# rbrito/deprecated-lame-mirror

Hardware: AMD Instinct MI355X
Metric: encoded audio seconds/sec (x real-time) at 44.1kHz stereo CBR128 (higher is better)
Workload: dtype f32

## Files before the change

### deprecated-lame-mirror_amd/csrc/lh_analysis.hip

```cpp
#include <stdint.h>
#include <math.h>

#ifdef LH_EMU
#include "hipemu.h"
#define LH_CONST static const
#else
#include <hip/hip_runtime.h>
#define LH_CONST __device__ static const
#endif

#if defined(LH_APROF) && !defined(LH_EMU)
__shared__ unsigned long long *lh_ap_base;
#define LH_PT(var) unsigned long long var = clock64()
#define LH_PA(idx, var) do { if (c.lane == 0) atomicAdd(&lh_ap_base[LH_NPROF * c.wave + 20 + (idx)], clock64() - var); } while (0)
#define LH_PC(idx) do { } while (0)
#endif
#define LH_CUSTOM_LDS "lh_lds_analysis.h"
#define LH_CUSTOM_SMP
#define LH_FZ_X(i) ((((i) >> 4) & 2) | (((i) >> 3) & 24) | (((i) >> 5) & 4))
#define LH_FZ(i) ((i) ^ LH_FZ_X(i))
#define LH_STAGE_IDX(i) LH_FZ(i)
#include "lh_static_tables.h"
#include "lh_dev_common.h"
#if !defined(LH_EMU)
#define LH_KRESTRICT __restrict__
#else
#define LH_KRESTRICT
#endif

#define LH_SPAN (lh_lds.work)
LH_DEVFN float
lh_smp(const LhCtx & c, int ch, int i)
{
    return LH_SPAN[ch * LH_BLKSIZE + LH_FZ(i)];
}

#include "lh_dev_psy_core.h"

struct LhGranuleAt {
    int     live;
    int     gr;
    long long at;
    long long frame_base;
};

LH_DEVFN LhGranuleAt
lh_granule_at(const LhStreamDesc & d, int g)
{
    LhGranuleAt o;
    int const nf = d.frame_end - d.frame_begin;
    int const fr = g / LH_NGR;
    o.live = g < LH_NGR * nf;
    o.gr = g - fr * LH_NGR;
    o.at = d.out_index + d.mid_rel + fr;
    o.frame_base = (long long) (576 * LH_NGR) * (d.frame_begin + fr) - LH_MF_START;
    return o;
}

LH_DEVFN LhStreamDesc
lh_desc_uniform(const LhStreamDesc * descs, int sidx)
{
    LhStreamDesc d = descs[sidx];
    d.pcm_l = lh_uni_ll(d.pcm_l);
    d.pcm_r = lh_uni_ll(d.pcm_r);
    d.pcm_base = lh_uni_ll(d.pcm_base);
    d.nsamples = lh_uni_ll(d.nsamples);
    d.out_index = lh_uni_ll(d.out_index);
    d.mid_rel = lh_uni_i(d.mid_rel);
    d.frame_begin = lh_uni_i(d.frame_begin);
    d.frame_end = lh_uni_i(d.frame_end);
    return d;
}

#ifdef LH_LSF
#define lh_attack_kernel lh_attack_kernel_lsf
#define lh_attack_scan_kernel lh_attack_scan_kernel_lsf
#define lh_analysis_kernel lh_analysis_kernel_lsf
#define lh_launch_analysis lh_launch_analysis_lsf
#define lh_emu_analysis lh_emu_analysis_lsf
#endif

#if defined(LH_APROF) && !defined(LH_EMU)
#define LH_AP_T0() unsigned long long ap_t = clock64()
#define LH_AP(k) do { unsigned long long const n_ = clock64(); if (c.lane == 0) atomicAdd(&aprof[64 * 0 + LH_NPROF * c.wave + (k)], n_ - ap_t); ap_t = n_; } while (0)
#else
#define LH_AP_T0() do { } while (0)
#define LH_AP(k) do { } while (0)
#endif
#define LH_FIR_SPAN 640

#ifndef LH_EMU
extern "C" __global__ void __launch_bounds__(64)
#else
void
#endif
lh_attack_kernel(const LhConfig * LH_KRESTRICT cfg, const int16_t * LH_KRESTRICT pcm, const float *pcmf, const LhStreamDesc * descs, LhMidFrame * frames,
                 int nstreams)
{
    __shared__ float span[2 * LH_FIR_SPAN];
    int const sidx = (int) blockIdx.y;
    LhCtx   c;
    c.cfg = cfg;
    c.T = nullptr;
    c.st = nullptr;
    c.pcm = pcm;
    c.pcmf = pcmf;
    c.d = lh_desc_uniform(descs, sidx);
    c.tid = (int) threadIdx.x;
    c.lane = c.tid;
    c.wave = 0;
    LhGranuleAt const ga = lh_granule_at(c.d, (int) blockIdx.x);
    if (!ga.live)
        return;
    int const lane = c.lane;
    int const n_chn_psy = (cfg->mode == LH_MODE_JOINT_STEREO) ? 4 : cfg->channels;
    int const bufbase = 576 + ga.gr * 576 - LH_FFTOFFSET;
    int const firbase = bufbase + 576 - 350 - LH_NSFIRLEN + 192;
    LhMidGr *mg = &frames[ga.at].small.gr[ga.gr];
    lh_stage_span < LH_FIR_SPAN, 64, 1 > (c, span, span + LH_FIR_SPAN, ga.frame_base + firbase);
    LH_WAVE_SYNC();
    {
        int const i0 = 9 * lane;
        float   x[2][30], y[2][9];
#pragma unroll
        for (int ch = 0; ch < 2; ch++)
#pragma unroll
            for (int t = 0; t < 30; t++)
                x[ch][t] = span[ch * LH_FIR_SPAN + i0 + t];
#pragma unroll
        for (int ch = 0; ch < 2; ch++)
#pragma unroll
            for (int m = 0; m < 9; m++) {
                float   sum1 = x[ch][m + 10], sum2 = 0.0;
#pragma unroll
                for (int j = 0; j < ((LH_NSFIRLEN - 1) / 2) - 1; j += 2) {
                    sum1 += lh_hp_fir[j] * (x[ch][m + j] + x[ch][m + LH_NSFIRLEN - j]);
                    sum2 += lh_hp_fir[j + 1] * (x[ch][m + j + 1] + x[ch][m + LH_NSFIRLEN - j - 1]);
                }
                y[ch][m] = sum1 + sum2;
            }
        LH_WAVE_SYNC();
#pragma unroll
        for (int ch = 0; ch < 2; ch++)
#pragma unroll
            for (int m = 0; m < 9; m++)
                span[ch * LH_FIR_SPAN + i0 + m] = y[ch][m];
    }
    LH_WAVE_SYNC();
    float   fl[9], fr[9];
#pragma unroll
    for (int k = 0; k < 9; k++) {
        fl[k] = span[lane + 64 * k];
        fr[k] = span[LH_FIR_SPAN + lane + 64 * k];
    }
    for (int chn = 0; chn < n_chn_psy; chn++) {
        uint32_t pk[8], pk8 = 0;
#pragma unroll
        for (int k = 0; k < 9; k++) {
            float const l = fl[k], r = fr[k];
            float const v = (chn == 0) ? l : (chn == 1) ? r : (chn == 2) ? l + r : l - r;
            if (k < 8)
                pk[k] = lh_f32_as_u32(lh_fabsf(v));
            else
                pk8 = lh_f32_as_u32(lh_fabsf(v));
        }
        {
            uint32_t const m8 = lh_wave_max8(pk);
            uint32_t const m9 = lh_wave_max_u32(pk8);
            if (lane < 9)
                mg->peak[chn][lane] = lh_u32_as_f32(lane == 8 ? m9 : m8);
        }
    }
}

#ifndef LH_SCAN_BLOCK
#define LH_SCAN_BLOCK 4
#endif
#ifndef LH_EMU
extern "C" __global__ void __launch_bounds__(64)
#else
void
#endif
lh_attack_scan_kernel(const LhConfig * LH_KRESTRICT cfg, const LhTables * LH_KRESTRICT T, const LhStreamDesc * descs, const LhStreamState * states,
                      LhMidFrame * frames, int nstreams)
{
    int const sidx = (int) blockIdx.x;
    int const lane = (int) threadIdx.x;
    LhStreamDesc const d = lh_desc_uniform(descs, sidx);
    int const nf = d.frame_end - d.frame_begin;
    if (nf <= 0)
        return;
    const LhStreamState *st = &states[sidx];
    int const n_chn_psy = lh_uni_i((cfg->mode == LH_MODE_JOINT_STEREO) ? 4 : cfg->channels);
    int const channels = lh_uni_i(cfg->channels), short_blocks = lh_uni_i(cfg->short_blocks);
    int const chn = lane >> 4, i = lane & 15, grp = lane & 48;
    int const mine = chn < n_chn_psy;
    float   le = st->last_en_subshort[chn][i < 9 ? i : 0];
    int     last_att = st->last_attacks[chn];
    float const thresh = T->attack_threshold[chn];
    int     bt_old0 = lh_uni_i(st->blocktype_old[0]), bt_old1 = lh_uni_i(st->blocktype_old[1]);
    int const ng = LH_NGR * nf;
    float   pk_blk[LH_SCAN_BLOCK];
#pragma unroll
    for (int j = 0; j < LH_SCAN_BLOCK; j++) {
        int const g = (j < ng) ? j : 0;
        pk_blk[j] = frames[d.out_index + d.mid_rel + g / LH_NGR].small.gr[g % LH_NGR].peak[chn][i < 9 ? i : 0];
    }
    for (int g0 = 0; g0 < ng; g0 += LH_SCAN_BLOCK) {
        float   pk_cur[LH_SCAN_BLOCK], ssf_blk[LH_SCAN_BLOCK];
        int     nsa_blk[LH_SCAN_BLOCK][4];
#pragma unroll
        for (int j = 0; j < LH_SCAN_BLOCK; j++) {
            int const gn = g0 + LH_SCAN_BLOCK + j, g = (gn < ng) ? gn : 0;
            pk_cur[j] = pk_blk[j];
            pk_blk[j] = frames[d.out_index + d.mid_rel + g / LH_NGR].small.gr[g % LH_NGR].peak[chn][i < 9 ? i : 0];
        }
#pragma unroll
        for (int j = 0; j < LH_SCAN_BLOCK; j++) {
            float const pk = pk_cur[j];
            float const fresh = pk < 1.0f ? 1.0f : pk;
            float const old = lh_shfl_f32(le, grp + ((i + 6) & 15)), older = lh_shfl_f32(le, grp + ((i + 4) & 15));
            float const got = lh_shfl_f32(fresh, grp + ((i - 3) & 15));
            float const e = (i < 3) ? old : got;
            float const e1 = lh_shfl_f32(e, grp + ((i - 1) & 15)), e0 = lh_shfl_f32(e, grp + ((i - 2) & 15));
            float const then = (i < 3) ? older : e0;
            float const ai = (i < 3) ? e / then : (e > then) ? e / then : (then > e * 10.0f) ? then / (e * 10.0f) : 0.0f;
            float const whole = e0 + e1 + e;
            int const tail_low = e * 6 < whole, mid_low = e1 * 6 < whole;
            uint64_t const over_all = lh_ballot(i < 12 && ai > thresh);
            unsigned const over = (unsigned) (over_all >> (16 * chn)) & 0xfffu;
            float   en_short[4];
            en_short[0] = lh_shfl_f32(whole, grp + 2);
            en_short[1] = lh_shfl_f32(whole, grp + 5);
            en_short[2] = lh_shfl_f32(whole, grp + 8);
            en_short[3] = lh_shfl_f32(whole, grp + 11);
            ssf_blk[j] = tail_low ? (mid_low ? 0.25f : 0.5f) : 1.0f;
            int    *nsa = nsa_blk[j];
            le = fresh;
            for (int gq = 0; gq < 4; gq++) {
                unsigned const bits = (over >> (3 * gq)) & 7u;
                nsa[gq] = bits ? ((bits & 1u) ? 1 : (bits & 2u) ? 2 : 3) : 0;
            }
            for (int q = 1; q < 4; q++) {
                float const u = en_short[q - 1];
                float const v = en_short[q];
                float const m = (u > v) ? u : v;
                if (m < 40000) {
                    if (u < 1.7f * v && v < 1.7f * u) {
                        if (q == 1 && nsa[0] <= nsa[q])
                            nsa[0] = 0;
                        nsa[q] = 0;
                    }
                }
            }
        }
#pragma unroll
        for (int j = 0; j < LH_SCAN_BLOCK; j++) {
            int const g = g0 + j;
            if (g >= ng)
                break;
            int const fr = g / LH_NGR, gr = g - fr * LH_NGR;
            LhMidGr *mg = &frames[d.out_index + d.mid_rel + fr].small.gr[gr];
            int    *nsa = nsa_blk[j];
            float const ssf = ssf_blk[j];
            int     uselong = 1;
            if (nsa[0] <= last_att)
                nsa[0] = 0;
            if (last_att == 3 || nsa[0] + nsa[1] + nsa[2] + nsa[3]) {
                uselong = 0;
                if (nsa[1] && nsa[0])
                    nsa[1] = 0;
                if (nsa[2] && nsa[1])
                    nsa[2] = 0;
                if (nsa[3] && nsa[2])
                    nsa[3] = 0;
            }
            if (!mine) {
                nsa[0] = nsa[1] = nsa[2] = nsa[3] = 0;
                uselong = 1;
            }
            else
                last_att = nsa[2];
            if (i == 5 || i == 8 || i == 11)
                mg->sub_short_factor[chn][(i - 5) / 3] = mine ? ssf : 1.0f;
            if (i < 4)
                mg->ns_attacks[chn][i] = (int8_t) (i == 0 ? nsa[0] : i == 1 ? nsa[1] : i == 2 ? nsa[2] : nsa[3]);
            {
                uint64_t const shorts = lh_ballot(!uselong);
                int const s0 = (int) (shorts & 1u), s1 = (int) ((shorts >> 16) & 1u), s23 = (int) ((shorts >> 32) & 0x10001u) != 0;
                int     ul0 = !s0, ul1 = (channels == 2) ? !s1 : 1;
                int     btd[2];
                if (s23)
                    ul0 = ul1 = 0;
                if (short_blocks == 1 && !(ul0 && ul1))
                    ul0 = ul1 = 0;
                if (short_blocks == 2)
                    ul0 = ul1 = 1;
                if (short_blocks == 3)
                    ul0 = ul1 = 0;
                for (int ch = 0; ch < 2; ch++) {
                    int     blocktype = LH_NORM_TYPE;
                    int     was = ch ? bt_old1 : bt_old0;
                    if (ch ? ul1 : ul0) {
                        if (was == LH_SHORT_TYPE)
                            blocktype = LH_STOP_TYPE;
                    }
                    else {
                        blocktype = LH_SHORT_TYPE;
                        if (was == LH_NORM_TYPE)
                            was = LH_START_TYPE;
                        if (was == LH_STOP_TYPE)
                            was = LH_SHORT_TYPE;
                    }
                    btd[ch] = was;
                    if (ch)
                        bt_old1 = lh_uni_i(blocktype);
                    else
                        bt_old0 = lh_uni_i(blocktype);
                }
                if (lane < 2) {
                    mg->uselong[lane] = (int8_t) (lane ? ul1 : ul0);
                    mg->block_type[lane] = (int8_t) (lane ? btd[1] : btd[0]);
                }
            }
        }
    }
}

template < int K1 > LH_DEVFN void
lh_fht_unit_fz(lh_f32x4 tw, float *fz, int u)
{
    constexpr int kx = K1 >> 1, k2 = K1 << 1, k3 = k2 + K1, k4 = k2 << 1;
    int const blk = u / kx, i = u - blk * kx;
    int const axis = (i == 0);
    int const lo = blk * k4 + i;
    int const hi = blk * k4 + (axis ? kx : K1 - i);
    int     al[4], ah[4];
    if (K1 == 4) {
        int const x = LH_FZ_X(lo);
#pragma unroll
        for (int j = 0; j < 4; j++) {
            al[j] = (lo + j * K1) ^ x;
            ah[j] = (hi + j * K1) ^ x;
        }
    }
    else if (K1 == 16) {
        int const x = LH_FZ_X(blk * k4);
#pragma unroll
        for (int j = 0; j < 4; j++) {
            al[j] = (lo + j * K1) ^ x ^ (j >= 2 ? 2 : 0);
            ah[j] = (hi + j * K1) ^ x ^ (j >= 2 ? 2 : 0);
        }
    }
    else if (K1 == 64) {
#pragma unroll
        for (int j = 0; j < 4; j++) {
            al[j] = (lo + j * K1) ^ LH_FZ_X(64 * j);
            ah[j] = (hi + j * K1) ^ (2 ^ LH_FZ_X(64 * j));
        }
    }
    else {
        int const xl = LH_FZ_X(lo), xh = LH_FZ_X(hi);
#pragma unroll
        for (int j = 0; j < 4; j++) {
            al[j] = (lo + j * K1) ^ xl;
            ah[j] = (hi + j * K1) ^ xh;
        }
    }
    float const p0 = fz[al[0]], p1 = fz[al[1]], p2 = fz[al[2]], p3 = fz[al[3]];
    float const q0 = fz[ah[0]], q1 = fz[ah[1]], q2 = fz[ah[2]], q3 = fz[ah[3]];
    float const s01 = p0 + p1, d01 = p0 - p1, s23 = p2 + p3, d23 = p2 - p3;
    float const r2 = (float) (LH_SQRT2 * q2), r3 = (float) (LH_SQRT2 * q3);
    float const t01 = q0 + q1, u01 = q0 - q1;
    float const a_l0 = s01 + s23, a_l1 = d01 + d23, a_l2 = s01 - s23, a_l3 = d01 - d23;
    float const a_h0 = t01 + r2, a_h1 = u01 + r3, a_h2 = t01 - r2, a_h3 = u01 - r3;
    LhRot const rq1 = lh_rot(tw.z, tw.w, p1, q1);
    LhRot const rq3 = lh_rot(tw.z, tw.w, p3, q3);
    float const le = p0 + rq1.along, lm = p0 - rq1.along;
    float const he = q0 + rq1.across, hm = q0 - rq1.across;
    float const l2e = p2 + rq3.along, l2m = p2 - rq3.along;
    float const h2e = q2 + rq3.across, h2m = q2 - rq3.across;
    LhRot const ra = lh_rot(tw.x, tw.y, l2e, h2m);
    LhRot const rb = lh_rot(tw.y, tw.x, h2e, l2m);
    fz[al[0]] = axis ? a_l0 : le + ra.along;
    fz[al[1]] = axis ? a_l1 : lm + rb.across;
    fz[al[2]] = axis ? a_l2 : le - ra.along;
    fz[al[3]] = axis ? a_l3 : lm - rb.across;
    fz[ah[0]] = axis ? a_h0 : he + rb.along;
    fz[ah[1]] = axis ? a_h1 : hm + ra.across;
    fz[ah[2]] = axis ? a_h2 : he - rb.along;
    fz[ah[3]] = axis ? a_h3 : hm - ra.across;
}

LH_DEVFN void
lh_fft_long_inplace(const LhCtx & c, float *x)
{
    const float *w = c.T->fft_window;
    int const lane = c.lane;
    float   o[2][8];
#pragma unroll
    for (int q = 0; q < 2; q++) {
        int const jj = lane + 64 * q;
        int const i = (int) lh_rev8((unsigned) jj);
        const float *xs = x + (i ^ LH_FZ_X(i));
        float   f0, f1, f2, f3, ww;
        f0 = w[i] * xs[0];
        ww = w[i + 0x200] * xs[0x200];
        f1 = f0 - ww;
        f0 = f0 + ww;
        f2 = w[i + 0x100] * xs[0x100];
        ww = w[i + 0x300] * xs[0x300];
        f3 = f2 - ww;
        f2 = f2 + ww;
        o[q][0] = f0 + f2;
        o[q][2] = f0 - f2;
        o[q][1] = f1 + f3;
        o[q][3] = f1 - f3;
        f0 = w[i + 0x001] * xs[0x001];
        ww = w[i + 0x201] * xs[0x201];
        f1 = f0 - ww;
        f0 = f0 + ww;
        f2 = w[i + 0x101] * xs[0x101];
        ww = w[i + 0x301] * xs[0x301];
        f3 = f2 - ww;
        f2 = f2 + ww;
        o[q][4] = f0 + f2;
        o[q][6] = f0 - f2;
        o[q][5] = f1 + f3;
        o[q][7] = f1 - f3;
    }
    {
        lh_f32x4 tw[4][2];
#pragma unroll
        for (int stage = 0; stage < 4; stage++) {
            int const kx = 2 << (2 * stage);
#pragma unroll
            for (int q = 0; q < 2; q++)
                tw[stage][q] = *(const lh_f32x4 *) c.T->fht_tw[stage][(lane + 64 * q) % kx];
        }
        LH_WAVE_SYNC_MEM();
#pragma unroll
        for (int q = 0; q < 2; q++) {
            int const at = 4 * (lane + 64 * q), xa = LH_FZ_X(at);
#pragma unroll
            for (int k = 0; k < 4; k++) {
                x[(at + k) ^ xa] = o[q][k];
                x[(at + k + LH_BLKSIZE / 2) ^ xa] = o[q][4 + k];
            }
        }
        LH_WAVE_SYNC_MEM();
#pragma unroll
        for (int q = 0; q < 2; q++)
            lh_fht_unit_fz < 4 > (tw[0][q], x, lane + 64 * q);
        LH_WAVE_SYNC_MEM();
#pragma unroll
        for (int q = 0; q < 2; q++)
            lh_fht_unit_fz < 16 > (tw[1][q], x, lane + 64 * q);
        LH_WAVE_SYNC_MEM();
#pragma unroll
        for (int q = 0; q < 2; q++)
            lh_fht_unit_fz < 64 > (tw[2][q], x, lane + 64 * q);
        LH_WAVE_SYNC_MEM();
#pragma unroll
        for (int q = 0; q < 2; q++)
            lh_fht_unit_fz < 256 > (tw[3][q], x, lane + 64 * q);
        LH_WAVE_SYNC_MEM();
    }
}

LH_DEVFN void
lh_fft_short_inplace(const LhCtx & c, float *x)
{
    const float *ws = c.T->fft_window_s;
    int const lane = c.lane;
    float   o[2][8];
#pragma unroll
    for (int q = 0; q < 2; q++) {
        int const t = lane + 64 * q, tt = t < 3 * (LH_BLKSIZE_S / 8) ? t : 0;
        int const b = tt >> 5, j = tt & 31;
        int const k = (576 / 3) * (b + 1);
        int const i = (int) lh_rev8((unsigned) (j << 2));
        float   f0, f1, f2, f3, w;
        f0 = ws[i] * x[LH_FZ(i + k)];
        w = ws[0x7f - i] * x[LH_FZ(i + k + 0x80)];
        f1 = f0 - w;
        f0 = f0 + w;
        f2 = ws[i + 0x40] * x[LH_FZ(i + k + 0x40)];
        w = ws[0x3f - i] * x[LH_FZ(i + k + 0xc0)];
        f3 = f2 - w;
        f2 = f2 + w;
        o[q][0] = f0 + f2;
        o[q][2] = f0 - f2;
        o[q][1] = f1 + f3;
        o[q][3] = f1 - f3;
        f0 = ws[i + 0x01] * x[LH_FZ(i + k + 0x01)];
        w = ws[0x7e - i] * x[LH_FZ(i + k + 0x81)];
        f1 = f0 - w;
        f0 = f0 + w;
        f2 = ws[i + 0x41] * x[LH_FZ(i + k + 0x41)];
        w = ws[0x3e - i] * x[LH_FZ(i + k + 0xc1)];
        f3 = f2 - w;
        f2 = f2 + w;
        o[q][4] = f0 + f2;
        o[q][6] = f0 - f2;
        o[q][5] = f1 + f3;
        o[q][7] = f1 - f3;
    }
    LH_WAVE_SYNC_MEM();
#pragma unroll
    for (int q = 0; q < 2; q++) {
        int const t = lane + 64 * q;
        if (t < 3 * (LH_BLKSIZE_S / 8)) {
            int const at = (t >> 5) * LH_BLKSIZE_S + 4 * (t & 31);
#pragma unroll
            for (int k = 0; k < 4; k++) {
                x[LH_FZ(at + k)] = o[q][k];
                x[LH_FZ(at + k + LH_BLKSIZE_S / 2)] = o[q][4 + k];
            }
        }
    }
    LH_WAVE_SYNC_MEM();
    for (int t = lane; t < 3 * (LH_BLKSIZE_S / 8); t += 64) {
        int const b = t >> 5, u = t & 31;
        lh_fht_unit_fz < 4 > (*(const lh_f32x4 *) c.T->fht_tw[0][u % 2], x + b * LH_BLKSIZE_S, u);
    }
    LH_WAVE_SYNC_MEM();
    for (int t = lane; t < 3 * (LH_BLKSIZE_S / 8); t += 64) {
        int const b = t >> 5, u = t & 31;
        lh_fht_unit_fz < 16 > (*(const lh_f32x4 *) c.T->fht_tw[1][u % 8], x + b * LH_BLKSIZE_S, u);
    }
    LH_WAVE_SYNC_MEM();
    for (int t = lane; t < 3 * (LH_BLKSIZE_S / 8); t += 64) {
        int const b = t >> 5, u = t & 31;
        lh_fht_unit_fz < 64 > (*(const lh_f32x4 *) c.T->fht_tw[2][u % 32], x + b * LH_BLKSIZE_S, u);
    }
    LH_WAVE_SYNC_MEM();
}

LH_DEVFN void
lh_an_spectra_short(const LhCtx & c, int w, int both, const float *wl, const float *wr, int first, float *out_own, float *out_ms)
{
    float const sqrt2_half = (float) (LH_SQRT2 * 0.5f);
    int const n = LH_BLKSIZE_S, h = n >> 1;
    for (int m = c.lane; m <= h; m += 64) {
        int const ire = first + m, iim = first + ((m == 0) ? 0 : (n - m));
        float const lre = wl[LH_FZ(ire)], lim = wl[LH_FZ(iim)], rre = wr[LH_FZ(ire)], rim = wr[LH_FZ(iim)];
        float const ore = w ? rre : lre, oim = w ? rim : lim;
        float const mre = (w ? lre - rre : lre + rre) * sqrt2_half, mim = (w ? lim - rim : lim + rim) * sqrt2_half;
        out_own[m] = (m == 0) ? ore * ore : (ore * ore + oim * oim) * 0.5f;
        if (both)
            out_ms[m] = (m == 0) ? mre * mre : (mre * mre + mim * mim) * 0.5f;
    }
}

LH_DEVFN void
lh_an_spectra(const LhCtx & c, int w, int own, int ms, float *work)
{
    float const sqrt2_half = (float) (LH_SQRT2 * 0.5f);
    const float *wl = work, *wr = work + LH_BLKSIZE;
    float   eo[9], em[9];
#pragma unroll
    for (int k = 0; k < 9; k++) {
        int const m0 = c.lane + 64 * k, m = m0 <= LH_BLKSIZE / 2 ? m0 : LH_BLKSIZE / 2;
        int const ire = m, iim = (m == 0) ? 0 : (LH_BLKSIZE - m);
        float const lre = wl[LH_FZ(ire)], lim = wl[LH_FZ(iim)], rre = wr[LH_FZ(ire)], rim = wr[LH_FZ(iim)];
        float const ore = w ? rre : lre, oim = w ? rim : lim;
        float const mre = (w ? lre - rre : lre + rre) * sqrt2_half, mim = (w ? lim - rim : lim + rim) * sqrt2_half;
        eo[k] = (m == 0) ? ore * ore : (ore * ore + oim * oim) * 0.5f;
        em[k] = (m == 0) ? mre * mre : (mre * mre + mim * mim) * 0.5f;
    }
    LH_SYNC_WG_LDS();
#pragma unroll
    for (int k = 0; k < 9; k++) {
        int const m = c.lane + 64 * k;
        if (m <= LH_BLKSIZE / 2) {
            if (own)
                work[w * LH_AN_ROW + m] = eo[k];
            if (ms)
                work[(w + 2) * LH_AN_ROW + m] = em[k];
        }
    }
}

#ifndef LH_EMU
extern "C" __global__ void __launch_bounds__(LH_NT, 6)
#else
void
#endif
lh_analysis_kernel(const LhConfig * LH_KRESTRICT cfg, const LhTables * LH_KRESTRICT T, const int16_t * LH_KRESTRICT pcm, const float *pcmf, const LhStreamDesc * descs,
                   LhMidFrame * frames, int nstreams, LhStreamState * states)
{
#if defined(LH_APROF) && !defined(LH_EMU)
    unsigned long long *aprof = &states[blockIdx.y].prof[0][0];
    if (threadIdx.x == 0)
        lh_ap_base = aprof;
#endif
    LH_AP_T0();
    LhLds & L = lh_lds;
    LhLds & P = L;
    float  *const work = L.work;
#define LH_AN_E(chn) (work + (chn) * LH_AN_ROW)
    int const sidx = (int) blockIdx.y;
    LhCtx   c;
    c.cfg = cfg;
    c.T = T;
    c.st = nullptr;
    c.pcm = pcm;
    c.pcmf = pcmf;
    c.d = lh_desc_uniform(descs, sidx);
    c.tid = (int) threadIdx.x;
    c.lane = c.tid & 63;
    c.wave = lh_uni_i(c.tid >> 6);
    LhGranuleAt const ga = lh_granule_at(c.d, (int) blockIdx.x);
    if (!ga.live)
        return;
    int const lane = c.lane, w = c.wave, gr = ga.gr;
    int const n_chn_psy = (cfg->mode == LH_MODE_JOINT_STEREO) ? 4 : cfg->channels;
    int const bufbase = 576 + gr * 576 - LH_FFTOFFSET;
    LhMidGr *mg = &frames[ga.at].small.gr[gr];
    if (c.tid < 2)
        L.uselong[c.tid] = mg->uselong[c.tid];
    LH_AP(0);
    lh_stage_span < LH_BLKSIZE, LH_NT > (c, LH_SPAN, LH_SPAN + LH_BLKSIZE, ga.frame_base + bufbase);
    LH_SYNC_WG_LDS();
    LH_AP(1);
    if (w < cfg->channels)
        lh_fft_long_inplace(c, work + w * LH_BLKSIZE);
    LH_SYNC_WG_LDS();
    LH_AP(2);
    lh_an_spectra(c, w, w < n_chn_psy, n_chn_psy == 4, work);
    LH_WAVE_SYNC_MEM();
    const float *stg_s3 = T->psy_l.s3;
    LH_WAVE_SYNC_MEM();
    LH_AP(3);
    LH_AP(4);
    {
        int const chn = (lane == 1) ? w + 2 : w;
        int const summing = lane < 3 && chn < n_chn_psy;
        int const loud = (lane == 2);
        float  *prod = (w == 0) ? P.eb : P.thr;
        const float *ew = T->ath_eql_w;
        const float *e = LH_AN_E(summing ? chn : w);
        float   acc = 0.0f;
        for (int h = 0; h < 2; h++) {
            int const j0 = 256 * h;
            LH_WAVE_SYNC_MEM();
#pragma unroll
            for (int q = 0; q < 4; q++) {
                int const j = j0 + lane + 64 * q;
                prod[j - j0] = LH_AN_E(w)[j] * ew[j];
            }
            LH_WAVE_SYNC_MEM();
            if (summing) {
                const lh_f32x4 *s4 = (const lh_f32x4 *) ((loud ? prod - j0 : e) + j0);
                lh_f32x4 a0 = s4[0], a1 = s4[1], a2 = s4[2], a3 = s4[3];
                if (h == 0 && !loud) {
                    a0.x = a0.y = a0.z = a0.w = 0.0f;
                    a1.x = a1.y = a1.z = a1.w = 0.0f;
                    a2.x = a2.y = a2.z = 0.0f;
                }
                for (int g = 0; g < 64; g += 4) {
                    int const n = (g + 4 < 64) ? g + 4 : g;
                    lh_f32x4 const b0 = s4[n], b1 = s4[n + 1], b2 = s4[n + 2], b3 = s4[n + 3];
#ifndef LH_EMU
                    asm volatile("v_add_f32 %0, %0, %1\n\tv_add_f32 %0, %0, %2\n\tv_add_f32 %0, %0, %3\n\tv_add_f32 %0, %0, %4\n\t"
                                 "v_add_f32 %0, %0, %5\n\tv_add_f32 %0, %0, %6\n\tv_add_f32 %0, %0, %7\n\tv_add_f32 %0, %0, %8\n\t"
                                 "v_add_f32 %0, %0, %9\n\tv_add_f32 %0, %0, %10\n\tv_add_f32 %0, %0, %11\n\tv_add_f32 %0, %0, %12\n\t"
                                 "v_add_f32 %0, %0, %13\n\tv_add_f32 %0, %0, %14\n\tv_add_f32 %0, %0, %15\n\tv_add_f32 %0, %0, %16"
                                 : "+v"(acc)
                                 : "v"(a0.x), "v"(a0.y), "v"(a0.z), "v"(a0.w), "v"(a1.x), "v"(a1.y), "v"(a1.z), "v"(a1.w),
                                   "v"(a2.x), "v"(a2.y), "v"(a2.z), "v"(a2.w), "v"(a3.x), "v"(a3.y), "v"(a3.z), "v"(a3.w));
#else
                    acc += a0.x; acc += a0.y; acc += a0.z; acc += a0.w;
                    acc += a1.x; acc += a1.y; acc += a1.z; acc += a1.w;
                    acc += a2.x; acc += a2.y; acc += a2.z; acc += a2.w;
                    acc += a3.x; acc += a3.y; acc += a3.z; acc += a3.w;
#endif
                    a0 = b0;
                    a1 = b1;
                    a2 = b2;
                    a3 = b3;
                }
            }
        }
        if (summing) {
            if (!loud) {
                acc += e[LH_BLKSIZE / 2];
                mg->tot_ener[chn] = acc;
            }
            else {
                acc = (float) (acc * LH_VO_SCALE);
                mg->loud[w] = acc;
            }
        }
        LH_WAVE_SYNC_MEM();
    }
    LH_SYNC_WG_LDS();
    LH_AP(5);
    {
        LhMidLong *ml = &frames[ga.at].lng;
        if (n_chn_psy == 4) {
            LhMaskChan const two[2] = {
                {w, LH_AN_E(w), &P.eb[w * 64], &P.thr[w * 64], nullptr, nullptr, &ml->m[gr][w]},
                {w + 2, LH_AN_E(w + 2), &P.eb[(w + 2) * 64], &P.thr[(w + 2) * 64], nullptr, nullptr, &ml->m[gr][w + 2]}
            };
            lh_compute_masking < 2, 1 > (c, 1, two, stg_s3);
        }
        else if (w < n_chn_psy) {
            LhMaskChan const one[1] = { {w, LH_AN_E(w), &P.eb[w * 64], &P.thr[w * 64], nullptr, nullptr, &ml->m[gr][w]} };
            lh_compute_masking < 1, 1 > (c, 1, one, stg_s3);
        }
    }
    LH_AP(6);
    int const any_short = lh_uni_i(!(L.uselong[0] && L.uselong[1]));
    if (!any_short)
        return;
    LH_SYNC_WG_LDS();
    lh_stage_span < LH_BLKSIZE, LH_NT > (c, LH_SPAN, LH_SPAN + LH_BLKSIZE, ga.frame_base + bufbase);
    LH_SYNC_WG_LDS();
    if (!L.uselong[w])
        lh_fft_short_inplace(c, work + w * LH_BLKSIZE);
    LH_SYNC_WG_LDS();
    for (int sblock = 0; sblock < 3; sblock++) {
        if (w < n_chn_psy && !L.uselong[w]) {
            LhMidShort *ms = &frames[ga.at].shrt;
            int const both = (n_chn_psy == 4);
            lh_an_spectra_short(c, w, both, work, work + LH_BLKSIZE, sblock * LH_BLKSIZE_S, L.eshort[w], L.eshort[w + 2 < 4 ? w + 2 : 3]);
            LH_WAVE_SYNC_MEM();
            if (both) {
                LhMaskChan const two[2] = {
                    {w, L.eshort[w], &P.eb[w * 64], &P.thr[w * 64], nullptr, nullptr, &ms->m[gr][sblock][w]},
                    {w + 2, L.eshort[w + 2], &P.eb[(w + 2) * 64], &P.thr[(w + 2) * 64], nullptr, nullptr, &ms->m[gr][sblock][w + 2]}
                };
                lh_compute_masking < 2, 1 > (c, 0, two, T->psy_s.s3);
            }
            else {
                LhMaskChan const one[1] = { {w, L.eshort[w], &P.eb[w * 64], &P.thr[w * 64], nullptr, nullptr, &ms->m[gr][sblock][w]} };
                lh_compute_masking < 1, 1 > (c, 0, one, T->psy_s.s3);
            }
        }
        LH_SYNC_WG_LDS();
    }
    LH_AP(7);
}

#ifndef LH_EMU
extern "C" int
lh_launch_analysis(const LhConfig * cfg, const LhTables * T, const int16_t * pcm, const float *pcmf, const LhStreamDesc * descs,
                   const LhStreamState * states, LhMidPools mid, int nstreams, int max_frames, void *stream)
{
    if (nstreams <= 0 || max_frames <= 0)
        return 0;
    dim3 const grid((unsigned) (LH_NGR * max_frames), (unsigned) nstreams);
    hipLaunchKernelGGL(lh_attack_kernel, grid, dim3(64), 0, (hipStream_t) stream, cfg, pcm, pcmf, descs, mid.frames, nstreams);
    hipLaunchKernelGGL(lh_attack_scan_kernel, dim3((unsigned) nstreams), dim3(64), 0, (hipStream_t) stream, cfg, T, descs, states,
                       mid.frames, nstreams);
    hipLaunchKernelGGL(lh_analysis_kernel, grid, dim3(LH_NT), 0, (hipStream_t) stream, cfg, T, pcm, pcmf, descs, mid.frames, nstreams,
                       (LhStreamState *) states);
    return (int) hipGetLastError();
}
#else
extern "C" int
lh_emu_analysis(const LhConfig * cfg, const LhTables * T, const int16_t * pcm, const float *pcmf, const LhStreamDesc * descs,
                const LhStreamState * states, const LhMidPools * pools, int nstreams, int max_frames)
{
    LhMidPools const mid = *pools;
    hipemu_dim3 grid = { (unsigned) (LH_NGR * max_frames), (unsigned) nstreams, 1 }, b64 = { 64, 1, 1 }, b128 = { LH_NT, 1, 1 };
    hipemu_dim3 grid1 = { (unsigned) nstreams, 1, 1 };
    hipemu_run(grid, b64,[=] () {
               lh_attack_kernel(cfg, pcm, pcmf, descs, mid.frames, nstreams);
               }
    );
    hipemu_run(grid1, b64,[=] () {
               lh_attack_scan_kernel(cfg, T, descs, states, mid.frames, nstreams);
               }
    );
    hipemu_run(grid, b128,[=] () {
               lh_analysis_kernel(cfg, T, pcm, pcmf, descs, mid.frames, nstreams, (LhStreamState *) states);
               }
    );
    return 0;
}
#endif
```

### deprecated-lame-mirror_amd/csrc/lh_lds_analysis.h

```cpp
#define LH_AN_ROW (LH_HBLKSIZE + 3)
struct LhLds {
    LhSmallState ss;
    LhCtxShared ctx;
    LhRgSlot rg[2];
    int     uselong[2];
    int     pad[2];
    float   work[4 * LH_AN_ROW] __attribute__((aligned(16)));
    float   eshort[4][LH_HBLKSIZE_S + 3] __attribute__((aligned(16)));
    float   eb[4 * 64];
    float   thr[4 * 64];
};
static_assert(4 * LH_AN_ROW >= 2 * LH_BLKSIZE, "both channels' spans fit the spectra's place");
__shared__ LhLds lh_lds __attribute__((aligned(16)));
```

Measured before the change: 84380.

## Fuse attack highpass into analysis kernel and split short-block pass into batched kernel

The separate attack kernel is removed. Its highpass FIR and peak computation now run inside the long analysis kernel, reusing the PCM span that kernel already stages, with the FIR output kept in an LDS union that overlaps the masking buffers. The short-block FFT and masking work moves to a new kernel that handles runs of 8 granules per workgroup, reads the uselong verdicts with a ballot, and skips granules where both channels use long blocks. This drops a PCM staging pass and a launch, and stops launching whole workgroups for granules that need no short-block work. In exchange, each short-block workgroup processes its granules serially, the analysis kernel now has to run before the attack scan, and the LDS layout changes.

Measured after the change: 84210. No clear change (-0.2%).

```diff
diff --git a/deprecated-lame-mirror_amd/csrc/lh_analysis.hip b/deprecated-lame-mirror_amd/csrc/lh_analysis.hip
--- a/deprecated-lame-mirror_amd/csrc/lh_analysis.hip
+++ b/deprecated-lame-mirror_amd/csrc/lh_analysis.hip
@@ -73,9 +73,9 @@
 }
 
 #ifdef LH_LSF
-#define lh_attack_kernel lh_attack_kernel_lsf
 #define lh_attack_scan_kernel lh_attack_scan_kernel_lsf
 #define lh_analysis_kernel lh_analysis_kernel_lsf
+#define lh_analysis_short_kernel lh_analysis_short_kernel_lsf
 #define lh_launch_analysis lh_launch_analysis_lsf
 #define lh_emu_analysis lh_emu_analysis_lsf
 #endif
@@ -87,73 +87,49 @@
 #define LH_AP_T0() do { } while (0)
 #define LH_AP(k) do { } while (0)
 #endif
-#define LH_FIR_SPAN 640
-
-#ifndef LH_EMU
-extern "C" __global__ void __launch_bounds__(64)
-#else
-void
-#endif
-lh_attack_kernel(const LhConfig * LH_KRESTRICT cfg, const int16_t * LH_KRESTRICT pcm, const float *pcmf, const LhStreamDesc * descs, LhMidFrame * frames,
-                 int nstreams)
-{
-    __shared__ float span[2 * LH_FIR_SPAN];
-    int const sidx = (int) blockIdx.y;
-    LhCtx   c;
-    c.cfg = cfg;
-    c.T = nullptr;
-    c.st = nullptr;
-    c.pcm = pcm;
-    c.pcmf = pcmf;
-    c.d = lh_desc_uniform(descs, sidx);
-    c.tid = (int) threadIdx.x;
-    c.lane = c.tid;
-    c.wave = 0;
-    LhGranuleAt const ga = lh_granule_at(c.d, (int) blockIdx.x);
-    if (!ga.live)
-        return;
-    int const lane = c.lane;
-    int const n_chn_psy = (cfg->mode == LH_MODE_JOINT_STEREO) ? 4 : cfg->channels;
-    int const bufbase = 576 + ga.gr * 576 - LH_FFTOFFSET;
-    int const firbase = bufbase + 576 - 350 - LH_NSFIRLEN + 192;
-    LhMidGr *mg = &frames[ga.at].small.gr[ga.gr];
-    lh_stage_span < LH_FIR_SPAN, 64, 1 > (c, span, span + LH_FIR_SPAN, ga.frame_base + firbase);
-    LH_WAVE_SYNC();
+#define LH_FIR_AT (576 - 350 - LH_NSFIRLEN + 192)
+#define LH_FIR_N 576
+static_assert(LH_FIR_AT + LH_FIR_N + LH_NSFIRLEN <= LH_BLKSIZE, "the filter's 597 samples lie inside the transforms' window");
+
+LH_DEVFN void
+lh_an_highpass(const LhCtx & c)
+{
+    int const lane = c.lane, w = c.wave;
+    float   (*fir)[LH_FIR_N] = lh_lds.u.fir;
     {
         int const i0 = 9 * lane;
-        float   x[2][30], y[2][9];
-#pragma unroll
-        for (int ch = 0; ch < 2; ch++)
-#pragma unroll
-            for (int t = 0; t < 30; t++)
-                x[ch][t] = span[ch * LH_FIR_SPAN + i0 + t];
-#pragma unroll
-        for (int ch = 0; ch < 2; ch++)
-#pragma unroll
-            for (int m = 0; m < 9; m++) {
-                float   sum1 = x[ch][m + 10], sum2 = 0.0;
-#pragma unroll
-                for (int j = 0; j < ((LH_NSFIRLEN - 1) / 2) - 1; j += 2) {
-                    sum1 += lh_hp_fir[j] * (x[ch][m + j] + x[ch][m + LH_NSFIRLEN - j]);
-                    sum2 += lh_hp_fir[j + 1] * (x[ch][m + j + 1] + x[ch][m + LH_NSFIRLEN - j - 1]);
-                }
-                y[ch][m] = sum1 + sum2;
-            }
-        LH_WAVE_SYNC();
-#pragma unroll
-        for (int ch = 0; ch < 2; ch++)
-#pragma unroll
-            for (int m = 0; m < 9; m++)
-                span[ch * LH_FIR_SPAN + i0 + m] = y[ch][m];
-    }
-    LH_WAVE_SYNC();
+        float   x[30], y[9];
+#pragma unroll
+        for (int t = 0; t < 30; t++)
+            x[t] = lh_smp(c, w, LH_FIR_AT + i0 + t);
+#pragma unroll
+        for (int m = 0; m < 9; m++) {
+            float   sum1 = x[m + 10], sum2 = 0.0;
+#pragma unroll
+            for (int j = 0; j < ((LH_NSFIRLEN - 1) / 2) - 1; j += 2) {
+                sum1 += lh_hp_fir[j] * (x[m + j] + x[m + LH_NSFIRLEN - j]);
+                sum2 += lh_hp_fir[j + 1] * (x[m + j + 1] + x[m + LH_NSFIRLEN - j - 1]);
+            }
+            y[m] = sum1 + sum2;
+        }
+#pragma unroll
+        for (int m = 0; m < 9; m++)
+            fir[w][i0 + m] = y[m];
+    }
+}
+
+LH_DEVFN void
+lh_an_peaks(const LhCtx & c, int n_chn_psy, LhMidGr * mg)
+{
+    int const lane = c.lane, w = c.wave;
+    float   (*fir)[LH_FIR_N] = lh_lds.u.fir;
     float   fl[9], fr[9];
 #pragma unroll
     for (int k = 0; k < 9; k++) {
-        fl[k] = span[lane + 64 * k];
-        fr[k] = span[LH_FIR_SPAN + lane + 64 * k];
-    }
-    for (int chn = 0; chn < n_chn_psy; chn++) {
+        fl[k] = fir[0][lane + 64 * k];
+        fr[k] = fir[1][lane + 64 * k];
+    }
+    for (int chn = w; chn < n_chn_psy; chn += 2) {
         uint32_t pk[8], pk8 = 0;
 #pragma unroll
         for (int k = 0; k < 9; k++) {
@@ -597,7 +573,7 @@
 #endif
     LH_AP_T0();
     LhLds & L = lh_lds;
-    LhLds & P = L;
+    LhLdsMask & P = L.u.m;
     float  *const work = L.work;
 #define LH_AN_E(chn) (work + (chn) * LH_AN_ROW)
     int const sidx = (int) blockIdx.y;
@@ -618,12 +594,14 @@
     int const n_chn_psy = (cfg->mode == LH_MODE_JOINT_STEREO) ? 4 : cfg->channels;
     int const bufbase = 576 + gr * 576 - LH_FFTOFFSET;
     LhMidGr *mg = &frames[ga.at].small.gr[gr];
-    if (c.tid < 2)
-        L.uselong[c.tid] = mg->uselong[c.tid];
     LH_AP(0);
     lh_stage_span < LH_BLKSIZE, LH_NT > (c, LH_SPAN, LH_SPAN + LH_BLKSIZE, ga.frame_base + bufbase);
     LH_SYNC_WG_LDS();
     LH_AP(1);
+    lh_an_highpass(c);
+    LH_SYNC_WG_LDS();
+    lh_an_peaks(c, n_chn_psy, mg);
+    LH_AP(13);
     if (w < cfg->channels)
         lh_fft_long_inplace(c, work + w * LH_BLKSIZE);
     LH_SYNC_WG_LDS();
@@ -712,34 +690,93 @@
         }
     }
     LH_AP(6);
-    int const any_short = lh_uni_i(!(L.uselong[0] && L.uselong[1]));
-    if (!any_short)
-        return;
-    LH_SYNC_WG_LDS();
-    lh_stage_span < LH_BLKSIZE, LH_NT > (c, LH_SPAN, LH_SPAN + LH_BLKSIZE, ga.frame_base + bufbase);
-    LH_SYNC_WG_LDS();
-    if (!L.uselong[w])
-        lh_fft_short_inplace(c, work + w * LH_BLKSIZE);
-    LH_SYNC_WG_LDS();
-    for (int sblock = 0; sblock < 3; sblock++) {
-        if (w < n_chn_psy && !L.uselong[w]) {
-            LhMidShort *ms = &frames[ga.at].shrt;
-            int const both = (n_chn_psy == 4);
-            lh_an_spectra_short(c, w, both, work, work + LH_BLKSIZE, sblock * LH_BLKSIZE_S, L.eshort[w], L.eshort[w + 2 < 4 ? w + 2 : 3]);
-            LH_WAVE_SYNC_MEM();
-            if (both) {
-                LhMaskChan const two[2] = {
-                    {w, L.eshort[w], &P.eb[w * 64], &P.thr[w * 64], nullptr, nullptr, &ms->m[gr][sblock][w]},
-                    {w + 2, L.eshort[w + 2], &P.eb[(w + 2) * 64], &P.thr[(w + 2) * 64], nullptr, nullptr, &ms->m[gr][sblock][w + 2]}
-                };
-                lh_compute_masking < 2, 1 > (c, 0, two, T->psy_s.s3);
-            }
-            else {
-                LhMaskChan const one[1] = { {w, L.eshort[w], &P.eb[w * 64], &P.thr[w * 64], nullptr, nullptr, &ms->m[gr][sblock][w]} };
-                lh_compute_masking < 1, 1 > (c, 0, one, T->psy_s.s3);
-            }
-        }
+}
+
+#ifndef LH_AS_RUN
+#define LH_AS_RUN 8
+#endif
+static_assert(LH_AS_RUN >= 1 && LH_AS_RUN <= 16, "two lanes and two bits of a word per granule of a run");
+#ifndef LH_EMU
+extern "C" __global__ void __launch_bounds__(LH_NT, 6)
+#else
+void
+#endif
+lh_analysis_short_kernel(const LhConfig * LH_KRESTRICT cfg, const LhTables * LH_KRESTRICT T, const int16_t * LH_KRESTRICT pcm, const float *pcmf,
+                         const LhStreamDesc * descs, LhMidFrame * frames, int nstreams, LhStreamState * states)
+{
+#if defined(LH_APROF) && !defined(LH_EMU)
+    unsigned long long *aprof = &states[blockIdx.y].prof[0][0];
+    if (threadIdx.x == 0)
+        lh_ap_base = aprof;
+#endif
+    LH_AP_T0();
+    LhLds & L = lh_lds;
+    LhLdsMask & P = L.u.m;
+    float  *const work = L.work;
+    int const sidx = (int) blockIdx.y;
+    int const w = lh_uni_i((int) threadIdx.x >> 6);
+    int const g0 = LH_AS_RUN * (int) blockIdx.x;
+    unsigned verdicts;
+    {
+        LhStreamDesc const d = lh_desc_uniform(descs, sidx);
+        int const ng = LH_NGR * (d.frame_end - d.frame_begin);
+        int const lane = (int) threadIdx.x & 63, j = lane >> 1, g = g0 + j;
+        int     ul = 1;
+        if (g0 >= ng)
+            return;
+        if (j < LH_AS_RUN && g < ng) {
+            LhGranuleAt const a = lh_granule_at(d, g);
+            ul = frames[a.at].small.gr[a.gr].uselong[lane & 1] != 0;
+        }
+        verdicts = (unsigned) lh_uni_i((int) (unsigned) lh_ballot(ul));
+    }
+#pragma unroll 1
+    for (int j = 0; j < LH_AS_RUN; j++) {
+        int const ulw = (int) (verdicts >> (2 * j + w)) & 1;
+        if (((verdicts >> (2 * j)) & 3u) == 3u)
+            continue;
+        LhCtx   c;
+        c.cfg = cfg;
+        c.T = T;
+        c.tid = (int) threadIdx.x;
+#ifndef LH_EMU
+        asm volatile("" : "+s"(c.T), "+s"(c.cfg), "+v"(c.tid));
+#endif
+        c.st = nullptr;
+        c.pcm = pcm;
+        c.pcmf = pcmf;
+        c.d = lh_desc_uniform(descs, sidx);
+        c.lane = c.tid & 63;
+        c.wave = w;
+        int const n_chn_psy = (c.cfg->mode == LH_MODE_JOINT_STEREO) ? 4 : c.cfg->channels;
+        LhGranuleAt const ga = lh_granule_at(c.d, g0 + j);
+        int const gr = ga.gr;
+        int const bufbase = 576 + gr * 576 - LH_FFTOFFSET;
+        lh_stage_span < LH_BLKSIZE, LH_NT > (c, LH_SPAN, LH_SPAN + LH_BLKSIZE, ga.frame_base + bufbase);
         LH_SYNC_WG_LDS();
+        if (!ulw)
+            lh_fft_short_inplace(c, work + w * LH_BLKSIZE);
+        LH_SYNC_WG_LDS();
+        for (int sblock = 0; sblock < 3; sblock++) {
+            if (w < n_chn_psy && !ulw) {
+                LhMidShort *ms = &frames[ga.at].shrt;
+                int const both = (n_chn_psy == 4);
+                lh_an_spectra_short(c, w, both, work, work + LH_BLKSIZE, sblock * LH_BLKSIZE_S, P.eshort[w], P.eshort[w + 2 < 4 ? w + 2 : 3]);
+                LH_WAVE_SYNC_MEM();
+                if (both) {
+                    LhMaskChan const two[2] = {
+                        {w, P.eshort[w], &P.eb[w * 64], &P.thr[w * 64], nullptr, nullptr, &ms->m[gr][sblock][w]},
+                        {w + 2, P.eshort[w + 2], &P.eb[(w + 2) * 64], &P.thr[(w + 2) * 64], nullptr, nullptr, &ms->m[gr][sblock][w + 2]}
+                    };
+                    lh_compute_masking < 2, 1 > (c, 0, two, c.T->psy_s.s3);
+                }
+                else {
+                    LhMaskChan const one[1] = { {w, P.eshort[w], &P.eb[w * 64], &P.thr[w * 64], nullptr, nullptr, &ms->m[gr][sblock][w]} };
+                    lh_compute_masking < 1, 1 > (c, 0, one, c.T->psy_s.s3);
+                }
+            }
+            LH_SYNC_WG_LDS();
+        }
     }
     LH_AP(7);
 }
@@ -752,11 +789,13 @@
     if (nstreams <= 0 || max_frames <= 0)
         return 0;
     dim3 const grid((unsigned) (LH_NGR * max_frames), (unsigned) nstreams);
-    hipLaunchKernelGGL(lh_attack_kernel, grid, dim3(64), 0, (hipStream_t) stream, cfg, pcm, pcmf, descs, mid.frames, nstreams);
+    dim3 const runs((unsigned) ((LH_NGR * max_frames + LH_AS_RUN - 1) / LH_AS_RUN), (unsigned) nstreams);
+    hipLaunchKernelGGL(lh_analysis_kernel, grid, dim3(LH_NT), 0, (hipStream_t) stream, cfg, T, pcm, pcmf, descs, mid.frames, nstreams,
+                       (LhStreamState *) states);
     hipLaunchKernelGGL(lh_attack_scan_kernel, dim3((unsigned) nstreams), dim3(64), 0, (hipStream_t) stream, cfg, T, descs, states,
                        mid.frames, nstreams);
-    hipLaunchKernelGGL(lh_analysis_kernel, grid, dim3(LH_NT), 0, (hipStream_t) stream, cfg, T, pcm, pcmf, descs, mid.frames, nstreams,
-                       (LhStreamState *) states);
+    hipLaunchKernelGGL(lh_analysis_short_kernel, runs, dim3(LH_NT), 0, (hipStream_t) stream, cfg, T, pcm, pcmf, descs, mid.frames,
+                       nstreams, (LhStreamState *) states);
     return (int) hipGetLastError();
 }
 #else
@@ -767,16 +806,17 @@
     LhMidPools const mid = *pools;
     hipemu_dim3 grid = { (unsigned) (LH_NGR * max_frames), (unsigned) nstreams, 1 }, b64 = { 64, 1, 1 }, b128 = { LH_NT, 1, 1 };
     hipemu_dim3 grid1 = { (unsigned) nstreams, 1, 1 };
-    hipemu_run(grid, b64,[=] () {
-               lh_attack_kernel(cfg, pcm, pcmf, descs, mid.frames, nstreams);
+    hipemu_dim3 runs = { (unsigned) ((LH_NGR * max_frames + LH_AS_RUN - 1) / LH_AS_RUN), (unsigned) nstreams, 1 };
+    hipemu_run(grid, b128,[=] () {
+               lh_analysis_kernel(cfg, T, pcm, pcmf, descs, mid.frames, nstreams, (LhStreamState *) states);
                }
     );
     hipemu_run(grid1, b64,[=] () {
                lh_attack_scan_kernel(cfg, T, descs, states, mid.frames, nstreams);
                }
     );
-    hipemu_run(grid, b128,[=] () {
-               lh_analysis_kernel(cfg, T, pcm, pcmf, descs, mid.frames, nstreams, (LhStreamState *) states);
+    hipemu_run(runs, b128,[=] () {
+               lh_analysis_short_kernel(cfg, T, pcm, pcmf, descs, mid.frames, nstreams, (LhStreamState *) states);
                }
     );
     return 0;
diff --git a/deprecated-lame-mirror_amd/csrc/lh_lds_analysis.h b/deprecated-lame-mirror_amd/csrc/lh_lds_analysis.h
--- a/deprecated-lame-mirror_amd/csrc/lh_lds_analysis.h
+++ b/deprecated-lame-mirror_amd/csrc/lh_lds_analysis.h
@@ -1,4 +1,9 @@
 #define LH_AN_ROW (LH_HBLKSIZE + 3)
+struct LhLdsMask {
+    float   eshort[4][LH_HBLKSIZE_S + 3] __attribute__((aligned(16)));
+    float   eb[4 * 64];
+    float   thr[4 * 64];
+};
 struct LhLds {
     LhSmallState ss;
     LhCtxShared ctx;
@@ -6,9 +11,11 @@
     int     uselong[2];
     int     pad[2];
     float   work[4 * LH_AN_ROW] __attribute__((aligned(16)));
-    float   eshort[4][LH_HBLKSIZE_S + 3] __attribute__((aligned(16)));
-    float   eb[4 * 64];
-    float   thr[4 * 64];
+    union {
+        LhLdsMask m;
+        float   fir[2][576];
+    } u __attribute__((aligned(16)));
 };
 static_assert(4 * LH_AN_ROW >= 2 * LH_BLKSIZE, "both channels' spans fit the spectra's place");
+static_assert(sizeof(LhLds) <= 163840 / 12, "twelve workgroups per CU");
 __shared__ LhLds lh_lds __attribute__((aligned(16)));
```
